# cvg/diffmvs

Measured on AMD Instinct MI355X. Metric: depth-maps/sec (640x512, 5 src views), higher is better.
Workload: dtype f32

## Files before the change

diffmvs_amd/_lib.py:

```python
from __future__ import annotations

import ctypes as C
import os

PKG = os.path.dirname(os.path.abspath(__file__))
HIP_LIB_PATH = os.environ.get("DMVS_LIB") or os.path.join(PKG, "libdmvs_hip.so")

ACT_NONE, ACT_RELU, ACT_SIGMOID, ACT_TANH, ACT_SILU = range(5)
IN_PLAIN, IN_UPSAMPLE2, IN_UNSHUFFLE2, IN_ZEROINSERT2 = range(4)
LAYOUT_NCHW, LAYOUT_NHWC, LAYOUT_NHWC_BF16, LAYOUT_NHWC_F16 = 0, 1, 2, 3
DTYPE_F32, DTYPE_BF16, DTYPE_F16, DTYPE_F32_PLAIN = 0, 1, 2, 3
ARITH_F32, ARITH_BF16, ARITH_SPLIT = 0, 1, 2
EW_DEPTH_TO_DISP, EW_DISP_TO_DEPTH = 0, 1

_P = C.c_void_p
_I = C.c_int32
_F = C.c_float


class Conv2dDesc(C.Structure):
    _fields_ = [
        ("in0", _P), ("in1", _P), ("mul0", _P), ("weight", _P), ("scale", _P), ("shift", _P),
        ("residual", _P), ("gru_z", _P), ("gru_h", _P), ("out", _P), ("gn_stats", _P), ("out_mul", _P),
        ("B", _I), ("c0", _I), ("c1", _I), ("Hin", _I), ("Win", _I), ("Hout", _I), ("Wout", _I),
        ("cout", _I), ("cout_pad", _I), ("kh", _I), ("kw", _I), ("stride", _I), ("pad_h", _I), ("pad_w", _I),
        ("in_mode", _I), ("act", _I), ("res_mode", _I), ("res_after_act", _I),
        ("out_layout", _I), ("out_cstride", _I), ("out_coffset", _I), ("gn_groups", _I), ("post_scale", _F),
        ("gate_cstride", _I), ("arith", _I), ("tune", _I), ("out_mul_c0", _I), ("in0_cstride", _I), ("weight_split", _P),
    ]


class Conv3dDesc(C.Structure):
    _fields_ = [
        ("in_", _P), ("weight", _P), ("scale", _P), ("shift", _P), ("residual", _P), ("out", _P),
        ("B", _I), ("cin", _I), ("cout", _I), ("cout_pad", _I),
        ("Din", _I), ("Hin", _I), ("Win", _I), ("Dout", _I), ("Hout", _I), ("Wout", _I),
        ("stride", _I), ("transposed", _I), ("act", _I), ("tune", _I),
    ]


class GetCostDesc(C.Structure):
    _fields_ = [
        ("ref", _P), ("src", _P), ("rt", _P), ("inv_depth", _P), ("confidence", _P), ("view_w", _P),
        ("disp_min", _P), ("disp_max", _P), ("out_cost", _P), ("out_samples", _P), ("worklist", _P),
        ("B", _I), ("S", _I), ("C", _I), ("G", _I), ("n", _I), ("H", _I), ("W", _I), ("vw_shift", _I),
        ("cost_cstride", _I), ("cost_coffset", _I), ("samp_cstride", _I), ("samp_coffset", _I),
        ("interval", _F), ("min_radius", _F), ("max_radius", _F), ("feat_dtype", _I), ("tune", _I),
    ]


SIGNATURES = {
    "dmvs_abi_version": [],
    "dmvs_conv2d_f32": [C.POINTER(Conv2dDesc), _P],
    "dmvs_featurenet_stem_f32": [_P, _P, _P, _P, _P, _P, _P, _P, _I, _I, _I, _I, _P],
    "dmvs_featurenet_stem3_f32": [_P, _P, _P, _P, _P, _P, _P, _P, _P, _P, _P, _I, _I, _I, _I, _P],
    "dmvs_featurenet_conv1_pair_f32": [_P, _P, _P, _P, _P, _P, _P, _P, _I, _I, _I, _I, _P],
    "dmvs_featurenet_fpn_tail_f32": [_P, _P, _P, _P, _P, _P, _I, _I, _I, _I, _P],
    "dmvs_conv2d_wgrad_workspace_f32": [C.POINTER(Conv2dDesc), C.POINTER(C.c_int64)],
    "dmvs_conv2d_wgrad_f32": [C.POINTER(Conv2dDesc), _P, _P, _P, _P, C.c_int64, _P],
    "dmvs_conv3d_f32": [C.POINTER(Conv3dDesc), _P],
    "dmvs_conv3d_wgrad_workspace_f32": [C.POINTER(Conv3dDesc), C.POINTER(C.c_int64)],
    "dmvs_conv3d_wgrad_f32": [C.POINTER(Conv3dDesc), _P, _P, _P, _P, C.c_int64, _P],
    "dmvs_compose_proj_f32": [_P, _P, _I, _I, _P],
    "dmvs_warp_volume_f32": [_P, _P, _P, _P, _I, _I, _I, _I, _I, _I, _I, _P],
    "dmvs_getcost_quad_f32": [C.POINTER(GetCostDesc), _P],
    "dmvs_warp_corr_init_quad_f32": [_P, _P, _P, _P, _P, _P, _I, _I, _I, _I, _I, _I, _I, _I, _I, _I, _I, _P],
    "dmvs_warp_corr_init_bwd_f32": [_P, _P, _P, _P, _P, _P, _P, _P, _I, _I, _I, _I, _I, _I, _I, _I, _I, _I, _P],
    "dmvs_getcost_bwd_f32": [C.POINTER(GetCostDesc), _P, _P, _P, _P],
    "dmvs_view_aggregate_bwd_f32": [_P, _P, _P, _P, _P, _P, _I, _I, _I, _I, _P],
    "dmvs_view_aggregate_f32": [_P, _P, _P, _I, _I, _I, _I, _P],
    "dmvs_sigmoid_max_d_f32": [_P, _P, _I, _I, _I, _P],
    "dmvs_depth_regress_f32": [_P, _P, _P, _P, _P, _P, _I, _I, _I, _P],
    "dmvs_convex_upsample_f32": [_P, _P, _P, _P, _P, _P, _I, _I, _I, _I, _P],
    "dmvs_mask_upsample4_f32": [_P, _P, _P, _F, _P, _P, _P, _P, _P, _I, _I, _I, _I, _I, _P],
    "dmvs_groupnorm_silu_f32": [_P, _P, _P, _P, _P, _P, _P, _I, _I, _I, _I, _F, _P],
    "dmvs_groupnorm_apply_f32": [_P, _P, _P, _P, _P, _P, _P, _I, _I, _I, _I, _F, _P],
# ... 96 lines not shown
```

diffmvs_amd/csrc/conv2d.hip:

```cpp
#include "conv2d_tiled.h"

namespace {

constexpr int kC11MaxCin = 64;

template <int NT, int OT, bool ACTX = false>
__global__ void __launch_bounds__(DMVS_BLOCK) conv1x1_px4_kernel(const dmvs_conv2d_desc d, int tiles_per_item) {
    constexpr int NW = NT * 16, WS = (NW % 32 == 0) ? NW + 16 : NW;
    __shared__ float s_w[kC11MaxCin * WS];
    DMVS_LDS_POISON(s_w);
    const int tid = threadIdx.x, lane = tid & 63, wave = tid >> 6;
    const int n = lane & 15, kq = lane >> 4;
    const int cin = d.c0 + d.c1, cin4 = (cin + 3) >> 2;
    const int HW = d.Hout * d.Wout;
    const int nbase = blockIdx.y * NW;
    for (int e = tid; e < cin4 * 4 * NW; e += DMVS_BLOCK) {
        const int k = e / NW, co = e - k * NW;
        s_w[k * WS + co] = (k < cin && nbase + co < d.cout_pad) ? d.weight[k * d.cout_pad + nbase + co] : 0.0f;
    }
    const int b = blockIdx.x / tiles_per_item, t = blockIdx.x - b * tiles_per_item;
    const int p = (t * 4 + wave) * 64 + 4 * n;
    const bool pok = p < HW;
    const int pcl = pok ? p : HW - 4;
    const float* in0b = d.in0 + (size_t)b * d.c0 * HW;
    const float* in1b = d.in1 ? d.in1 + (size_t)b * d.c1 * HW : d.in0;
    __syncthreads();

    f32x4 acc[4][NT];
#pragma unroll
    for (int r = 0; r < 4; ++r)
#pragma unroll
        for (int j = 0; j < NT; ++j) acc[r][j] = f32x4{0.0f, 0.0f, 0.0f, 0.0f};
    auto load = [&](int c) -> f32x4 {
        int ci = 4 * c + kq;
        ci = ci < cin ? ci : cin - 1;
        const float* src = ci < d.c0 ? in0b + (size_t)ci * HW : in1b + (size_t)(ci - d.c0) * HW;
        return *reinterpret_cast<const f32x4*>(src + pcl);
    };
    auto mma = [&](int c, const f32x4& x) {
        const bool ok = pok && 4 * c + kq < cin;
        const float* wp = s_w + (4 * c + kq) * WS + n;
        float xv[4];
#pragma unroll
        for (int r = 0; r < 4; ++r) xv[r] = ok ? x[r] : 0.0f;
#pragma unroll
        for (int nt = 0; nt < NT; ++nt) {
            const float aw = wp[nt * 16];
#pragma unroll
// ... 26 lines not shown
    for (int nt = 0; nt < NT; ++nt) {
        f32x4 y[4], res[4];
#pragma unroll
        for (int j = 0; j < 4; ++j) {
            const int cg = nbase + nt * 16 + 4 * kq + j;
            res[j] = f32x4{0.0f, 0.0f, 0.0f, 0.0f};
            if (resb && cg < d.cout) {
                if (rup) {
                    typedef float f32x2 __attribute__((ext_vector_type(2)));
                    const f32x2 rv = *reinterpret_cast<const f32x2*>(resb + (size_t)cg * rplane + rpix);
                    res[j] = f32x4{rv[0], rv[0], rv[1], rv[1]};
                } else {
                    res[j] = *reinterpret_cast<const f32x4*>(resb + (size_t)cg * HW + p);
                }
            }
        }
#pragma unroll
        for (int j = 0; j < 4; ++j) {
            const int cg = nbase + nt * 16 + 4 * kq + j;
            const bool okc = cg < d.cout;
            const float sc = d.scale ? d.scale[okc ? cg : 0] : 1.0f, sh = d.shift ? d.shift[okc ? cg : 0] : 0.0f;
#pragma unroll
            for (int r = 0; r < 4; ++r) y[j][r] = acc[r][nt][j] * sc + sh;
            if (!d.res_after_act) y[j] += res[j];
            if constexpr (ACTX) {
#pragma unroll
                for (int r = 0; r < 4; ++r) y[j][r] = dmvs_act(y[j][r], d.act);
            } else if (d.act == DMVS_ACT_RELU) {
#pragma unroll
                for (int r = 0; r < 4; ++r) y[j][r] = fmaxf(y[j][r], 0.0f);
            }
            y[j] *= d.post_scale;
            if (d.res_after_act) y[j] += res[j];
        }
        if constexpr (OT != DMVS_DTYPE_F32) {
            const int c0o = nbase + nt * 16 + 4 * kq;
            uint16_t* const ob = reinterpret_cast<uint16_t*>(d.out) + ((size_t)b * HW + p) * d.out_cstride + d.out_coffset + c0o;
#pragma unroll
            for (int r = 0; r < 4; ++r)
#pragma unroll
                for (int j = 0; j < 4; ++j)
                    if (c0o + j < d.cout) ob[(size_t)r * d.out_cstride + j] = dmvs_to_x16<OT>(y[j][r]);
        } else if (d.out_layout == DMVS_LAYOUT_NCHW) {
            float* const outb = d.out + ((size_t)b * d.out_cstride + d.out_coffset) * HW + p;
#pragma unroll
            for (int j = 0; j < 4; ++j) {
// ... 14 lines not shown
                        if (c0o + j < d.cout) ob[(size_t)r * d.out_cstride + j] = y[j][r];
                }
            }
        }
    }
}

static bool conv1x1_px4_ok(const dmvs_conv2d_desc& d) {
    if (d.kh != 1 || d.kw != 1 || d.stride != 1 || d.pad_h || d.pad_w || d.in_mode != DMVS_IN_PLAIN) return false;
    if (d.mul0 || d.gru_z || d.gn_stats || d.out_mul || d.in0_cstride || (d.tune & DMVS_TUNE_1X1_TILED)) return false;
    if (d.act > DMVS_ACT_RELU && (d.cout_pad > 16 || d.out_layout != DMVS_LAYOUT_NCHW)) return false;
    if (d.c0 + d.c1 > kC11MaxCin || d.cout_pad > 144 || (d.Wout & 3)) return false;
    if (d.res_mode == DMVS_IN_UPSAMPLE2 && ((d.Hout | d.Wout) & 1)) return false;
    if ((((uintptr_t)d.in0 | (uintptr_t)d.in1 | (uintptr_t)d.residual) & 15) != 0) return false;
    if (d.out_layout == DMVS_LAYOUT_NCHW && ((uintptr_t)d.out & 15)) return false;
    return true;
}

template <int NT>
static int launch_conv1x1_px4(const dmvs_conv2d_desc& d, hipStream_t st, int ngroups) {
    const int HW = d.Hout * d.Wout;
    const int tiles = (HW + 255) / 256;
    dim3 grid((unsigned)(tiles * d.B), (unsigned)ngroups), block(DMVS_BLOCK);
    if (d.out_layout == DMVS_LAYOUT_NHWC_BF16) hipLaunchKernelGGL((conv1x1_px4_kernel<NT, DMVS_DTYPE_BF16>), grid, block, 0, st, d, tiles);
    else if (d.out_layout == DMVS_LAYOUT_NHWC_F16) hipLaunchKernelGGL((conv1x1_px4_kernel<NT, DMVS_DTYPE_F16>), grid, block, 0, st, d, tiles);
    else hipLaunchKernelGGL((conv1x1_px4_kernel<NT, DMVS_DTYPE_F32>), grid, block, 0, st, d, tiles);
    return dmvs_launch_status();
}

static int conv1x1_px4(const dmvs_conv2d_desc& d, hipStream_t st) {
    if (d.act > DMVS_ACT_RELU) {
        const int HW = d.Hout * d.Wout, tiles = (HW + 255) / 256;
        hipLaunchKernelGGL((conv1x1_px4_kernel<1, DMVS_DTYPE_F32, true>), dim3((unsigned)(tiles * d.B)), dim3(DMVS_BLOCK), 0, st, d, tiles);
        return dmvs_launch_status();
    }
    const int ntiles = (d.cout_pad + 15) / 16;
    const int maxnt = d.residual ? 2 : 4;
    const int ngroups = (ntiles + maxnt - 1) / maxnt;
    const int nt = (ntiles + ngroups - 1) / ngroups;
    switch (nt) {
        case 1: return launch_conv1x1_px4<1>(d, st, ngroups);
        case 2: return launch_conv1x1_px4<2>(d, st, ngroups);
        case 3: return launch_conv1x1_px4<3>(d, st, ngroups);
        default: return launch_conv1x1_px4<4>(d, st, ngroups);
    }
}

template <int KH, int KW, int S, bool V16>
__global__ void __launch_bounds__(DMVS_BLOCK) conv2d_wgrad_kernel(const dmvs_conv2d_desc d, const float* __restrict__ gout,
                                                                  float* __restrict__ ws, int want_bias, int tiles_x, int tiles_y) {
    constexpr int T = KH * KW, CK = 8;
    constexpr int TW = 15 * S + KW, TH = 15 * S + KH;
    constexpr int SLACK = V16 ? (4 - ((KW - 1) / 2) % 4) % 4 : 0;
    constexpr int TWL = V16 ? (SLACK + TW + 3) / 4 * 4 : TW;
    constexpr int PLANE = pad16mod32(TH * TWL);
    constexpr int GROW = V16 ? 260 : 257;
    constexpr int NTN = (CK * T + 1 + 15) / 16;
    constexpr int IN_IT = ((V16 ? CK * PLANE / 4 : CK * PLANE) + DMVS_BLOCK - 1) / DMVS_BLOCK;
    constexpr int G_IT = ((V16 ? 16 * GROW / 4 : 16 * GROW) + DMVS_BLOCK - 1) / DMVS_BLOCK;
    __shared__ __attribute__((aligned(16))) float lds[CK * PLANE + 16 * GROW];
    DMVS_LDS_POISON(lds);
    float* s_in = lds;
    float* s_g = lds + CK * PLANE;

    const int tid = threadIdx.x, lane = tid & 63, wave = tid >> 6;
    const int m = lane & 15, kq = lane >> 4;
    const int c0 = blockIdx.y * CK, cobase = blockIdx.z * 16;
    const int cin = d.c0 + d.c1;
// ... 190 lines not shown
    g.floats = (long)g.gx * g.gy * g.gz * g.ntn * 256;
    return g;
}

template <int KH, int KW, int S>
int launch_wgrad(const dmvs_conv2d_desc& d, const float* gout, float* gw, float* gb, float* ws, hipStream_t st) {
    const int tiles_x = (d.Wout + 15) / 16, tiles_y = (d.Hout + 15) / 16;
    const WgradGrid g = wgrad_grid(d);
    const bool v16 = !(d.tune & DMVS_TUNE_PIECES4) && d.in_mode == DMVS_IN_PLAIN && !d.mul0 && (d.Win & 3) == 0 && (d.Wout & 3) == 0 &&
                     d.pad_w == (KW - 1) / 2 && (((uintptr_t)d.in0 | (uintptr_t)d.in1 | (uintptr_t)gout) & 15) == 0;
    if (v16)
        hipLaunchKernelGGL((conv2d_wgrad_kernel<KH, KW, S, true>), dim3(g.gx, g.gy, g.gz), dim3(DMVS_BLOCK), 0, st, d, gout, ws,
                           gb ? 1 : 0, tiles_x, tiles_y);
    else
    hipLaunchKernelGGL((conv2d_wgrad_kernel<KH, KW, S, false>), dim3(g.gx, g.gy, g.gz), dim3(DMVS_BLOCK), 0, st, d, gout, ws,
                       gb ? 1 : 0, tiles_x, tiles_y);
    hipLaunchKernelGGL((conv2d_wgrad_reduce_kernel<KH * KW>), dim3(g.ntn * 16, g.gy, g.gz), dim3(DMVS_BLOCK), 0, st, ws, gw, gb,
                       g.gx, g.gy, d.c0 + d.c1, d.cout, (d.tune & DMVS_TUNE_WGRAD_ACCUMULATE) ? 1 : 0);
    return dmvs_launch_status();
}

}

extern "C" int dmvs_conv2d_f32(const dmvs_conv2d_desc* dp, void* stream) {
    if (!dp) return DMVS_EINVAL;
    const dmvs_conv2d_desc& d = *dp;
    hipStream_t st = (hipStream_t)stream;
    if (d.cout_pad % 8 || d.cout > d.cout_pad || d.B <= 0 || !d.in0 || !d.weight || !d.out) return DMVS_EINVAL;
    if ((uintptr_t)d.weight & 15) return DMVS_EINVAL;
    if (d.c1 > 0 && (!d.in1 || d.in_mode != DMVS_IN_PLAIN)) return DMVS_EINVAL;
    if (d.mul0 && d.in_mode != DMVS_IN_PLAIN) return DMVS_EINVAL;
    if (d.in_mode == DMVS_IN_UNSHUFFLE2 && (d.c0 % 4)) return DMVS_EINVAL;
    if ((d.in_mode == DMVS_IN_UPSAMPLE2 || d.in_mode == DMVS_IN_ZEROINSERT2) && ((d.Hin | d.Win) & 1)) return DMVS_EINVAL;
    if (d.gru_z && (!d.gru_h || d.act != DMVS_ACT_TANH)) return DMVS_EINVAL;
    if (d.gate_cstride < 0 || (d.gate_cstride && d.in_mode != DMVS_IN_PLAIN)) return DMVS_EINVAL;
    if (d.in0_cstride < 0 || (d.in0_cstride && (d.in_mode != DMVS_IN_PLAIN || d.in0_cstride < d.c0))) return DMVS_EINVAL;
    if (d.out_mul && (d.out_mul_c0 < 0 || d.out_mul_c0 >= d.cout || d.gn_stats)) return DMVS_EINVAL;
    if (d.gn_stats && (d.gn_groups != 4 || d.cout % 4)) return DMVS_EINVAL;
    if (d.arith != DMVS_ARITH_F32 && d.arith != DMVS_ARITH_BF16 && d.arith != DMVS_ARITH_SPLIT) return DMVS_EINVAL;
    const int eh = (d.Hin + 2 * d.pad_h - d.kh) / d.stride + 1, ew = (d.Win + 2 * d.pad_w - d.kw) / d.stride + 1;
    if (eh != d.Hout || ew != d.Wout) return DMVS_EINVAL;
    if ((long)(d.c0 + d.c1) * d.Hin * d.Win * (d.in_mode == DMVS_IN_UNSHUFFLE2 ? 4 : 1) >= (1L << 31)) return DMVS_EINVAL;
    if (d.out_layout < DMVS_LAYOUT_NCHW || d.out_layout > DMVS_LAYOUT_NHWC_F16) return DMVS_EINVAL;
    if (d.out_layout >= DMVS_LAYOUT_NHWC_BF16 && (d.gru_z || d.gn_stats)) return DMVS_EINVAL;
    const int ocs = d.out_cstride > d.cout ? d.out_cstride : d.cout;
    if ((long)d.Hout * d.Wout >= (1L << 24) || ocs >= (1 << 24) || (long)ocs * d.Hout * d.Wout >= (1L << 31)) return DMVS_EINVAL;
    const int key = d.kh * 100 + d.kw * 10 + d.stride;
    switch (key) {
        case 111:
            return conv1x1_px4_ok(d) ? conv1x1_px4(d, st) : dmvs_detail::launch_conv2d_111(d, st);
        case 331: return dmvs_detail::launch_conv2d_331(d, st);
        case 332: return dmvs_detail::launch_conv2d_332(d, st);
        case 552: return dmvs_detail::launch_conv2d_552(d, st);
        case 551: return dmvs_detail::launch_conv2d_551(d, st);
        case 771: return dmvs_detail::launch_conv2d_771(d, st);
        case 151: return dmvs_detail::launch_conv2d_151(d, st);
        case 511: return dmvs_detail::launch_conv2d_511(d, st);
        default: return DMVS_EINVAL;
    }
}

static int wgrad_check(const dmvs_conv2d_desc& d) {
    if (d.cout_pad % 8 || d.cout > d.cout_pad || d.B <= 0 || !d.in0) return DMVS_EINVAL;
    if (d.c1 > 0 && (!d.in1 || d.in_mode != DMVS_IN_PLAIN)) return DMVS_EINVAL;
    if (d.mul0 && d.in_mode != DMVS_IN_PLAIN) return DMVS_EINVAL;
    if (d.in0_cstride || d.gate_cstride || d.out_mul) return DMVS_EINVAL;
    const int eh = (d.Hin + 2 * d.pad_h - d.kh) / d.stride + 1, ew = (d.Win + 2 * d.pad_w - d.kw) / d.stride + 1;
    if (eh != d.Hout || ew != d.Wout) return DMVS_EINVAL;
    return 0;
}

extern "C" int dmvs_conv2d_wgrad_workspace_f32(const dmvs_conv2d_desc* dp, int64_t* bytes) {
    if (!dp || !bytes) return DMVS_EINVAL;
    if (int rc = wgrad_check(*dp)) return rc;
    *bytes = (int64_t)wgrad_grid(*dp).floats * 4;
    return 0;
}

extern "C" int dmvs_conv2d_wgrad_f32(const dmvs_conv2d_desc* dp, const float* grad_out, float* gw, float* gb, float* workspace,
                                     int64_t workspace_bytes, void* stream) {
    if (!dp || !grad_out || !gw || !workspace) return DMVS_EINVAL;
    const dmvs_conv2d_desc& d = *dp;
// ... 16 lines not shown
```

diffmvs_amd/csrc/misc.hip:

```cpp
#include "dmvs_common.h"

extern "C" int dmvs_abi_version(void) { return DMVS_ABI_VERSION; }

__device__ static void build_cam(const float* pm, double (&P)[4][4]) {
    const float* E = pm;
    const float* K = pm + 16;
    for (int i = 0; i < 4; ++i)
        for (int j = 0; j < 4; ++j) P[i][j] = (double)E[i * 4 + j];
    for (int i = 0; i < 3; ++i)
        for (int j = 0; j < 4; ++j) {
            double a = 0.0;
            for (int k = 0; k < 3; ++k) a += (double)K[i * 4 + k] * (double)E[k * 4 + j];
            P[i][j] = a;
        }
}

__global__ void compose_proj_kernel(const float* __restrict__ proj, float* __restrict__ out, int B, int V) {
    const int S = V - 1;
    const int idx = blockIdx.x * blockDim.x + threadIdx.x;
    if (idx >= B * S) return;
    const int b = idx / S, s = idx % S;
    double R[4][4], A[4][8];
    build_cam(proj + ((size_t)b * V) * 32, R);
    for (int i = 0; i < 4; ++i)
// ... 217 lines not shown
    }
    __syncthreads();
    if (threadIdx.x == 0) {
        double a = 0.0, c = 0.0;
        for (int w = 0; w < DMVS_BLOCK / 64; ++w) {
            a += red[0][w];
            c += red[1][w];
        }
        dmvs_gn_accumulate(&stats[2 * bg], 0, a);
        dmvs_gn_accumulate(&stats[2 * bg], 1, c);
    }
}

constexpr int kGnPerLane = 16;

template <bool VEC>
__global__ void __launch_bounds__(DMVS_BLOCK)
gn_apply_kernel(const float* __restrict__ x, const float* __restrict__ gamma, const float* __restrict__ beta,
                const float* __restrict__ scale_shift, const float* __restrict__ residual, float* __restrict__ y,
                const double* __restrict__ stats, int C, int HW, int groups, float eps) {
    __shared__ float s_ab[2];
    const int bc = blockIdx.y;
    if (threadIdx.x == 0) {
        const int b = bc / C, c = bc % C;
        const int cg = C / groups;
        const int g = c / cg;
        const double n = (double)cg * HW;
        double s1, s2;
        dmvs_gn_read_pair(&stats[2 * (b * groups + g)], s1, s2);
        const double mean = s1 / n;
        double var = s2 / n - mean * mean;
        var = var < 0.0 ? 0.0 : var;
        const float rstd = (float)(1.0 / sqrt(var + (double)eps));
        float A = rstd * gamma[c];
        float Bc = beta[c] - (float)mean * A;
        if (scale_shift) {
            const float sc = scale_shift[(long)b * 2 * C + c] + 1.0f, sh = scale_shift[(long)b * 2 * C + C + c];
            A *= sc;
            Bc = Bc * sc + sh;
        }
        s_ab[0] = A;
        s_ab[1] = Bc;
    }
    __syncthreads();
    const float A = s_ab[0], Bc = s_ab[1];
    const long base = (long)bc * HW;
    const int i0 = blockIdx.x * (DMVS_BLOCK * kGnPerLane);
    if constexpr (VEC) {
        typedef float f32x4 __attribute__((ext_vector_type(4)));
#pragma unroll
        for (int k = 0; k < kGnPerLane / 4; ++k) {
            const int i = i0 + (k * DMVS_BLOCK + threadIdx.x) * 4;
            if (i < HW) {
                f32x4 v = *reinterpret_cast<const f32x4*>(x + base + i);
#pragma unroll
                for (int j = 0; j < 4; ++j) {
                    const float t = fmaf(v[j], A, Bc);
                    v[j] = t * dmvs_sigmoid(t);
                }
                if (residual) v += *reinterpret_cast<const f32x4*>(residual + base + i);
                *reinterpret_cast<f32x4*>(y + base + i) = v;
            }
        }
    } else {
#pragma unroll 4
        for (int k = 0; k < kGnPerLane; ++k) {
            const int i = i0 + k * DMVS_BLOCK + threadIdx.x;
            if (i < HW) {
                float v = fmaf(x[base + i], A, Bc);
                v = v * dmvs_sigmoid(v);
                if (residual) v += residual[base + i];
                y[base + i] = v;
            }
        }
    }
}

static void launch_gn_apply(const float* x, const float* gamma, const float* beta, const float* scale_shift, const float* residual,
                            float* y, const double* stats, int B, int C, int HW, int groups, float eps, hipStream_t st) {
    const dim3 grid(dmvs_ceil_div(HW, DMVS_BLOCK * kGnPerLane), (unsigned)(B * C));
    const bool vec = HW % 4 == 0 && (((uintptr_t)x | (uintptr_t)y | (uintptr_t)residual) & 15) == 0;
    if (vec) hipLaunchKernelGGL((gn_apply_kernel<true>), grid, dim3(DMVS_BLOCK), 0, st, x, gamma, beta, scale_shift, residual, y, stats, C, HW, groups, eps);
    else hipLaunchKernelGGL((gn_apply_kernel<false>), grid, dim3(DMVS_BLOCK), 0, st, x, gamma, beta, scale_shift, residual, y, stats, C, HW, groups, eps);
}

extern "C" int dmvs_groupnorm_silu_f32(const float* x, const float* gamma, const float* beta, const float* scale_shift,
                                       const float* residual, float* y, double* stats, int32_t B, int32_t C, int32_t HW,
                                       int32_t groups, float eps, void* stream) {
    if (!x || !y || !stats || groups <= 0 || C % groups) return DMVS_EINVAL;
    hipStream_t st = (hipStream_t)stream;
    hipError_t e = hipMemsetAsync(stats, 0, sizeof(double) * 2 * B * groups, st);
    if (e != hipSuccess) return (int)e;
    const long per_group = (long)(C / groups) * HW;
// ... 173 lines not shown
```

diffmvs_amd/engine.py:

```python
from __future__ import annotations

import math
import os
from typing import Callable, Dict, List, Optional

import torch
import torch.nn.functional as F

from . import ops as K
from .ops import Ops, PackedConv, pack_conv2d, pack_conv3d

_RATIOS = [4, 2, 1]
_MULTS = [(1,), (1, 2), (1, 2, 4)]


def _bn(sd, p):
    return {k: sd[f"{p}.{k}"] for k in ("weight", "bias", "running_mean", "running_var")}


def _cw(sd, p, **kw):
    return pack_conv2d(sd[p + ".conv.weight"], sd.get(p + ".conv.bias"),
                       bn=_bn(sd, p + ".bn") if (p + ".bn.weight") in sd else None, **kw)


# ... 174 lines not shown

    def reset(self, B):
        self.buf = self.bufs.get(B)
        if self.buf is None:
            self.buf = self.bufs[B] = torch.zeros(self.SLOTS, B * 8, dtype=torch.float64, device=self.ops.device)
        else:
            self.buf.zero_()
        self.next = 0

    def slot(self):
        if self.next >= self.SLOTS:
            raise RuntimeError("GroupNorm statistics arena exhausted")
        s = self.buf[self.next]
        self.next += 1
        return s


def run_resblock(o: Ops, arena: GnArena, rb, x0, x1=None, scale_shift=None):
    st1, st2 = arena.slot(), arena.slot()
    h = o.conv2d(rb["c1"], x0, x1, gn_stats=st1)
    h = o.groupnorm_apply(h, rb["g1"][0], rb["g1"][1], 4, st1, scale_shift=scale_shift, out=h)
    h2 = o.conv2d(rb["c2"], h, gn_stats=st2)
    if rb["res"] is not None:
        res = o.conv2d(rb["res"], x0, x1)
    else:
        assert x1 is None
        res = x0
    return o.groupnorm_apply(h2, rb["g2"][0], rb["g2"][1], 4, st2, residual=res, out=h2)


def run_unet(o: Ops, arena: GnArena, ub, E, ctx_part, hidden, ss_of):
    x = o.conv2d(ub.init_enc, E, residual=ctx_part)
    r = x
    skips = []
    L = len(ub.mults)
    for i, (blk, ds) in enumerate(ub.downs):
        x = run_resblock(o, arena, blk, x, None, ss_of(blk))
        skips.append(x)
        x = o.conv2d(ds, x, in_mode=(K.IN_UNSHUFFLE2 if i < L - 1 else K.IN_PLAIN))
    hidden = run_gru(o, ub.gru, hidden, x)
    x = run_resblock(o, arena, ub.mid, hidden, None, None)
    for i, (blk, us) in enumerate(ub.ups):
        x = run_resblock(o, arena, blk, x, skips.pop(), ss_of(blk))
        x = o.conv2d(us, x, in_mode=(K.IN_UPSAMPLE2 if i < L - 1 else K.IN_PLAIN))
    x = run_resblock(o, arena, ub.final, x, r, ss_of(ub.final))
    delta = o.conv2d(ub.final_conv, x)
# ... 355 lines not shown
```

diffmvs_amd/ops.py:

```python
from __future__ import annotations

import ctypes as C
import os
from dataclasses import dataclass
from typing import Optional

import torch

from . import _lib
from ._lib import (ACT_NONE, ACT_RELU, ACT_SIGMOID, ACT_SILU, ACT_TANH, ARITH_BF16, ARITH_F32, ARITH_SPLIT, DTYPE_BF16, DTYPE_F16, DTYPE_F32, IN_PLAIN,
                   IN_UNSHUFFLE2, IN_UPSAMPLE2, IN_ZEROINSERT2, LAYOUT_NCHW, LAYOUT_NHWC, LAYOUT_NHWC_BF16, LAYOUT_NHWC_F16)

CONV_ARITH = {"fp32": ARITH_F32, "bf16": ARITH_BF16, "split": ARITH_SPLIT}
FEATURE_DTYPES = {"fp32": torch.float32, "bf16": torch.bfloat16, "fp16": torch.float16}
_DTYPE_CODE = {torch.float32: DTYPE_F32, torch.bfloat16: DTYPE_BF16, torch.float16: DTYPE_F16}
_NHWC_LAYOUT = {torch.float32: LAYOUT_NHWC, torch.bfloat16: LAYOUT_NHWC_BF16, torch.float16: LAYOUT_NHWC_F16}


def _round_up(x: int, m: int) -> int:
    return (x + m - 1) // m * m


@dataclass
class PackedConv:
# ... 109 lines not shown
def bump_weights_generation() -> None:
    _weights_generation[0] += 1


BWD_INTERLEAVED_DEFAULT = 1


def _env_tune():
    e = os.environ.get
    t2 = _lib.tune_tile_wx(int(e("DMVS_CONV_WX", "0"))) | _lib.tune_tile_mt(int(e("DMVS_CONV_MT", "0")))
    t2 |= _lib.TUNE_NO_WALK if e("DMVS_CONV_WALK") == "0" else 0
    t2 |= _lib.TUNE_PIECES4 if e("DMVS_CONV_V16") == "0" else 0
    t2 |= _lib.TUNE_NO_LEAN if e("DMVS_CONV_LEAN") == "0" else 0
    t2 |= _lib.TUNE_1X1_TILED if e("DMVS_CONV1X1_PX4") == "0" else 0
    t2 |= {"0": _lib.TUNE_NO_TALL, "1": _lib.TUNE_TALL}.get(e("DMVS_CONV_TALL"), 0)
    t2 |= _lib.TUNE_SPLIT_ALL if e("DMVS_CONV_SPLIT_ALL") == "1" else 0
    t2 |= _lib.tune_xcd_group(int(e("DMVS_CONV_XCD", "0")))
    t3 = (_lib.TUNE3D_PIECES4 if e("DMVS_CONV3D_V16") == "0" else 0) | (_lib.TUNE3D_S2_DIRECT if e("DMVS_CONV3D_S2") == "direct" else 0)
    t3 |= _lib.TUNE3D_NO_PAIR if e("DMVS_CONV3D_PAIR") == "0" else 0
    t3 |= _lib.tune3d_xcd_group(int(e("DMVS_CONV3D_XCD", "0")))
    return {"conv2d": t2, "conv3d": t3, "stem": (_lib.TUNE_PIECES4 if e("DMVS_STEM_V16") == "0" else 0) | _lib.tune_xcd_group(int(e("DMVS_STEM_XCD", "0"))) | (_lib.TUNE_STEM_EXACT if e("DMVS_STEM_EXACT") == "1" else 0),
            "sweep": _lib.TUNE_SWEEP_GLOBAL if e("DMVS_PLANE_SWEEP") == "quad" else 0,
            "bwd_gather": e("DMVS_GETCOST_BWD") == "gather",
            "bwd_il": e("DMVS_BWD_INTERLEAVED", "%d" % BWD_INTERLEAVED_DEFAULT) == "1"}


class Ops:
    _bindings = {}

    def __init__(self, lib: _lib.Lib, device):
        self.lib = lib
        self.device = torch.device(device)
        self.tune = _env_tune()
        self.timers = None
        self.conv_arith = ARITH_F32
        self.debug_fill = None
        self.getcost_hook = None

    def with_conv_arith(self, arith: int) -> "Ops":
        import copy
        o = copy.copy(self)
        o.conv_arith = arith
        return o

    def _call(self, name, *args):
        if self.timers is not None and name in self.timers:
            st, en = torch.cuda.Event(enable_timing=True), torch.cuda.Event(enable_timing=True)
            st.record()
            self.lib.call(name, *args)
            en.record()
            self.timers[name].append((st, en))
        else:
            self.lib.call(name, *args)

    @classmethod
    def for_device(cls, device) -> "Ops":
        device = torch.device(device)
        if device.type != "cuda":
            raise _lib.DmvsError(
                f"diffmvs_amd runs on MI355X only (got device '{device}'); there is no CPU path. "
                "Move the model and inputs to a HIP device.")
        if device.index is None:
            device = torch.device("cuda", torch.cuda.current_device())
        lib = _lib.hip_lib()
        key = (lib.path, device.index)
        o = cls._bindings.get(key)
        if o is None:
            o = cls._bindings[key] = cls(lib, device)
        return o

    def stream(self):
        if self.device.type == "cuda":
            return C.c_void_p(torch.cuda.current_stream(self.device).cuda_stream)
        return None
# ... 14 lines not shown
        dt = ts[0].dtype
        for t in ts:
            if t.dtype not in _DTYPE_CODE or t.dtype != dt or not t.is_contiguous() or t.device != self.device:
                raise _lib.DmvsError(f"expected contiguous fp32 / bf16 / fp16 feature tensors of one dtype on {self.device}, got "
                                     f"{t.dtype} contiguous={t.is_contiguous()} on {t.device}")
        return _DTYPE_CODE[dt]

    def _chk(self, *ts):
        for t in ts:
            if t is None:
                continue
            if t.dtype != torch.float32 or not t.is_contiguous() or t.device != self.device:
                raise _lib.DmvsError(f"expected contiguous fp32 tensor on {self.device}, got {t.dtype} "
                                     f"contiguous={t.is_contiguous()} on {t.device}")

    def _chk_typed(self, what, *pairs):
        for t, dt in pairs:
            if t is not None and (t.dtype != dt or not t.is_contiguous() or t.device != self.device):
                raise _lib.DmvsError(f"{what}: expected a contiguous {dt} tensor on {self.device}, got {t.dtype} on {t.device}")

    def conv2d(self, pc: PackedConv, x0, x1=None, *, mul0=None, in_mode=IN_PLAIN, act=ACT_NONE, residual=None,
               res_mode=IN_PLAIN, res_after_act=False, post_scale=1.0, gru_z=None, gru_h=None, out=None,
               out_layout=LAYOUT_NCHW, out_cstride=None, out_coffset=0, gn_stats=None, gn_groups=4, out_dtype=torch.float32,
               gate_cstride=0, arith=None, tune=None, out_mul=None, out_mul_c0=0, in0_cstride=0):
        if in0_cstride:
            if (x0.dtype != torch.float32 or x0.device != self.device or x0.stride(1) != x0.shape[2] * x0.shape[3] or
                    x0.stride(0) != in0_cstride * x0.shape[2] * x0.shape[3] or x0.stride(3) != 1 or in_mode != IN_PLAIN):
                raise _lib.DmvsError("in0_cstride: x0 must be a channel slice of a contiguous [B,in0_cstride,H,W] tensor, plain input mode")
        self._chk(out_mul)
        if gate_cstride:
            self._chk(*(() if in0_cstride else (x0,)), x1, residual, gru_h)
            for t in (mul0, gru_z):
                if t is not None and (t.dtype != torch.float32 or t.device != self.device or t.stride(1) != t.shape[2] * t.shape[3] or
                                      t.stride(0) != gate_cstride * t.shape[2] * t.shape[3] or t.stride(3) != 1):
                    raise _lib.DmvsError("gate_cstride: mul0 / gru_z must be channel slices of a contiguous [B,gate_cstride,H,W] tensor")
        else:
            self._chk(*(() if in0_cstride else (x0,)), x1, mul0, residual, gru_z, gru_h)
        if out_dtype != torch.float32:
            if out_layout != LAYOUT_NHWC or out is not None:
                raise _lib.DmvsError("16-bit outputs are channel-last feature tensors allocated by conv2d")
            out_layout = _NHWC_LAYOUT[out_dtype]
        else:
            self._chk(out)
        if gn_stats is not None and (gn_stats.dtype != torch.float64 or gn_stats.numel() < x0.shape[0] * gn_groups * 2):
            raise _lib.DmvsError("gn_stats must be float64 with B*groups*2 elements")
        B = x0.shape[0]
        if in_mode == IN_PLAIN:
# ... 4 lines not shown
            c0, Hin, Win = x0.shape[1] * 4, x0.shape[2] // 2, x0.shape[3] // 2
        c1 = 0 if x1 is None else x1.shape[1]
        assert c0 + c1 == pc.cin, (c0, c1, pc.cin)
        kh, kw = pc.k
        Hout = (Hin + 2 * pc.pad[0] - kh) // pc.stride + 1
        Wout = (Win + 2 * pc.pad[1] - kw) // pc.stride + 1
        if out_cstride is None:
            out_cstride = pc.cout
        if out is None:
            shape = (B, out_cstride, Hout, Wout) if out_layout == LAYOUT_NCHW else (B, Hout, Wout, out_cstride)
            out = self.empty(*shape, dtype=out_dtype)
        arith = self.conv_arith if arith is None else arith
        wsplit = split_weights(pc) if (arith == ARITH_SPLIT and kh * kw > 1 and out_layout in (LAYOUT_NCHW, LAYOUT_NHWC)) else None
        d = _lib.Conv2dDesc(
            weight_split=_ptr(wsplit),
            in0=_ptr(x0), in1=_ptr(x1), mul0=_ptr(mul0), weight=_ptr(pc.weight), scale=_ptr(pc.scale),
            shift=_ptr(pc.shift), residual=_ptr(residual), gru_z=_ptr(gru_z), gru_h=_ptr(gru_h), out=_ptr(out),
            gn_stats=_ptr(gn_stats), gn_groups=(gn_groups if gn_stats is not None else 0), B=B, c0=c0, c1=c1, Hin=Hin, Win=Win, Hout=Hout, Wout=Wout, cout=pc.cout, cout_pad=pc.cout_pad,
            kh=kh, kw=kw, stride=pc.stride, pad_h=pc.pad[0], pad_w=pc.pad[1], in_mode=in_mode, act=act,
            res_mode=res_mode, res_after_act=int(res_after_act), out_layout=out_layout, out_cstride=out_cstride,
            out_coffset=out_coffset, post_scale=post_scale, gate_cstride=gate_cstride,
            arith=arith, tune=(self.tune["conv2d"] if tune is None else tune),
            out_mul=_ptr(out_mul), out_mul_c0=out_mul_c0, in0_cstride=in0_cstride)
        self._call("dmvs_conv2d_f32", C.byref(d), self.stream())
        if self.timers is not None and "dmvs_conv2d_f32" in self.timers:
            self.timers.setdefault("_conv2d_flops", []).append(2.0 * B * Hout * Wout * pc.cout * pc.cin * kh * kw)
            self.timers.setdefault("_conv2d_shape", []).append((B, pc.cin, pc.cout, kh, kw, pc.stride, Hout, Wout, in_mode, int(mul0 is not None)))
            nb = sum(t.numel() * t.element_size() for t in (x0, x1, mul0, residual, gru_z, gru_h, out_mul) if t is not None)
            self.timers.setdefault("_conv2d_bytes", []).append(nb + B * Hout * Wout * pc.cout * out.element_size())
        return out

    def featurenet_stem(self, pc0: PackedConv, pc1: PackedConv, x, tune=None):
        if isinstance(x, (list, tuple)):
            self._chk(*x)
            Bv, cin, H, W = x[0].shape
            y = self.empty(len(x) * Bv, 8, H, W)
            for v, xv in enumerate(x):
                self._stem_launch(pc0, pc1, xv, y[v * Bv:(v + 1) * Bv], tune)
            return y
        self._chk(x)
        N, cin, H, W = x.shape
        y = self.empty(N, 8, H, W)
        self._stem_launch(pc0, pc1, x, y, tune)
        return y

    def _stem_launch(self, pc0: PackedConv, pc1: PackedConv, x, y, tune=None):
        N, cin, H, W = x.shape
# ... 683 lines not shown
```

include/dmvs.h:

```cpp
#ifndef DMVS_H
#define DMVS_H

#include <stdint.h>

#ifdef __cplusplus
extern "C" {
#endif

#define DMVS_ABI_VERSION 4
#define DMVS_EINVAL (-22)

enum { DMVS_ACT_NONE = 0, DMVS_ACT_RELU = 1, DMVS_ACT_SIGMOID = 2, DMVS_ACT_TANH = 3, DMVS_ACT_SILU = 4 };
enum { DMVS_IN_PLAIN = 0, DMVS_IN_UPSAMPLE2 = 1 , DMVS_IN_UNSHUFFLE2 = 2 ,
       DMVS_IN_ZEROINSERT2 = 3  };
enum { DMVS_LAYOUT_NCHW = 0, DMVS_LAYOUT_NHWC = 1,
       DMVS_LAYOUT_NHWC_BF16 = 2, DMVS_LAYOUT_NHWC_F16 = 3 };
enum { DMVS_DTYPE_F32 = 0 , DMVS_DTYPE_BF16 = 1, DMVS_DTYPE_F16 = 2 ,
       DMVS_DTYPE_F32_PLAIN = 3  };

int dmvs_abi_version(void);

#define DMVS_ARITH_F32 0
#define DMVS_ARITH_BF16 1
#define DMVS_ARITH_SPLIT 2
// ... 23 lines not shown
    double* gn_stats;
    const float* out_mul;
    int32_t B, c0, c1;
    int32_t Hin, Win;
    int32_t Hout, Wout;
    int32_t cout, cout_pad;
    int32_t kh, kw, stride, pad_h, pad_w;
    int32_t in_mode, act;
    int32_t res_mode;
    int32_t res_after_act;
    int32_t out_layout, out_cstride, out_coffset;
    int32_t gn_groups;
    float post_scale;
    int32_t gate_cstride;
    int32_t arith;
    int32_t tune;
    int32_t out_mul_c0;
    int32_t in0_cstride;
    const void* weight_split;
} dmvs_conv2d_desc;

int dmvs_conv2d_f32(const dmvs_conv2d_desc* d, void* stream);

int dmvs_featurenet_stem_f32(const float* x, const float* w0, const float* scale0, const float* shift0, const float* w1,
                             const float* scale1, const float* shift1, float* y, int32_t N, int32_t H, int32_t W, int32_t tune,
                             void* stream);

int dmvs_featurenet_stem3_f32(const float* x, const float* w0, const float* scale0, const float* shift0, const float* w1,
                              const float* scale1, const float* shift1, const float* w2, const float* scale2, const float* shift2,
                              float* y, int32_t N, int32_t H, int32_t W, int32_t tune, void* stream);

int dmvs_featurenet_conv1_pair_f32(const float* x, const void* wsplit1, const float* scale1, const float* shift1, const void* wsplit2,
                                   const float* scale2, const float* shift2, float* y, int32_t N, int32_t H, int32_t W, int32_t tune,
                                   void* stream);

int dmvs_featurenet_fpn_tail_f32(const float* c2, const float* c3, const float* w_inner, const float* b_inner, const void* wsplit_out,
                                 float* y, int32_t N, int32_t H, int32_t W, int32_t tune, void* stream);

#define DMVS_TUNE_WGRAD_ACCUMULATE 0x1000
int dmvs_conv2d_wgrad_workspace_f32(const dmvs_conv2d_desc* d, int64_t* bytes);
int dmvs_conv2d_wgrad_f32(const dmvs_conv2d_desc* d, const float* grad_out, float* gw, float* gb, float* workspace,
                          int64_t workspace_bytes, void* stream);

typedef struct dmvs_conv3d_desc {
    const float* in;
    const float* weight;
// ... 211 lines not shown
```

Measured before the change: 1547.

## Fuse GroupNorm+SiLU of residual branch into the 1x1 shortcut conv epilogue

Adds a GN-aware variant of the 1x1 conv kernel that builds per-channel GroupNorm affine coefficients in shared memory and applies GN+SiLU to the residual operand in the epilogue, writing in place over h2. In the residual block this replaces a separate shortcut conv, a groupnorm_apply pass and a residual-add read/write with a single kernel, saving one full feature-map round trip through memory. The fused path is enabled by default through a tune flag and only taken when alignment and shape checks pass. In exchange the epilogue recomputes GN coefficients per workgroup and each element pays a sigmoid.

Result: no change. 1553, median of 4 (+0.4%).

```diff
diff --git a/diffmvs_amd/_lib.py b/diffmvs_amd/_lib.py
--- a/diffmvs_amd/_lib.py
+++ b/diffmvs_amd/_lib.py
@@ -30,6 +30,10 @@
     ]
 
 
+class GnOperand(C.Structure):
+    _fields_ = [("stats", _P), ("gamma", _P), ("beta", _P), ("scale_shift", _P), ("groups", _I), ("eps", _F)]
+
+
 class Conv3dDesc(C.Structure):
     _fields_ = [
         ("in_", _P), ("weight", _P), ("scale", _P), ("shift", _P), ("residual", _P), ("out", _P),
@@ -52,6 +56,7 @@
 SIGNATURES = {
     "dmvs_abi_version": [],
     "dmvs_conv2d_f32": [C.POINTER(Conv2dDesc), _P],
+    "dmvs_conv2d_gn_f32": [C.POINTER(Conv2dDesc), C.POINTER(GnOperand), _P],
     "dmvs_featurenet_stem_f32": [_P, _P, _P, _P, _P, _P, _P, _P, _I, _I, _I, _I, _P],
     "dmvs_featurenet_stem3_f32": [_P, _P, _P, _P, _P, _P, _P, _P, _P, _P, _P, _I, _I, _I, _I, _P],
     "dmvs_featurenet_conv1_pair_f32": [_P, _P, _P, _P, _P, _P, _P, _P, _I, _I, _I, _I, _P],
diff --git a/diffmvs_amd/csrc/conv2d.hip b/diffmvs_amd/csrc/conv2d.hip
--- a/diffmvs_amd/csrc/conv2d.hip
+++ b/diffmvs_amd/csrc/conv2d.hip
@@ -1,11 +1,14 @@
 #include "conv2d_tiled.h"
+#include "dmvs_gn.h"
 
 namespace {
 
 constexpr int kC11MaxCin = 64;
 
-template <int NT, int OT, bool ACTX = false>
-__global__ void __launch_bounds__(DMVS_BLOCK) conv1x1_px4_kernel(const dmvs_conv2d_desc d, int tiles_per_item) {
+struct conv_no_gn {};
+template <int NT, int OT, bool ACTX = false, bool GNR = false>
+__global__ void __launch_bounds__(DMVS_BLOCK) conv1x1_px4_kernel(const dmvs_conv2d_desc d, int tiles_per_item,
+                                                                 const std::conditional_t<GNR, dmvs_gn_operand, conv_no_gn> gn) {
     constexpr int NW = NT * 16, WS = (NW % 32 == 0) ? NW + 16 : NW;
     __shared__ float s_w[kC11MaxCin * WS];
     DMVS_LDS_POISON(s_w);
@@ -24,6 +27,14 @@
     const int pcl = pok ? p : HW - 4;
     const float* in0b = d.in0 + (size_t)b * d.c0 * HW;
     const float* in1b = d.in1 ? d.in1 + (size_t)b * d.c1 * HW : d.in0;
+    [[maybe_unused]] const float* s_gn = nullptr;
+    if constexpr (GNR) {
+        __shared__ float s_gn_tab[2 * DMVS_GN_TABLE];
+        static_assert(NW <= DMVS_GN_TABLE, "one table slot per output channel of the workgroup");
+        DMVS_LDS_POISON(s_gn_tab);
+        dmvs_gn_fill_table(s_gn_tab, gn, b, nbase, NW, d.cout, HW, tid);
+        s_gn = s_gn_tab;
+    }
     __syncthreads();
 
     f32x4 acc[4][NT];
@@ -96,6 +107,11 @@
             const float sc = d.scale ? d.scale[okc ? cg : 0] : 1.0f, sh = d.shift ? d.shift[okc ? cg : 0] : 0.0f;
 #pragma unroll
             for (int r = 0; r < 4; ++r) y[j][r] = acc[r][nt][j] * sc + sh;
+            if constexpr (GNR) {
+                const float ga = s_gn[nt * 16 + 4 * kq + j], gb = s_gn[DMVS_GN_TABLE + nt * 16 + 4 * kq + j];
+#pragma unroll
+                for (int r = 0; r < 4; ++r) res[j][r] = okc ? dmvs_gn_silu(res[j][r], ga, gb) : 0.0f;
+            }
             if (!d.res_after_act) y[j] += res[j];
             if constexpr (ACTX) {
 #pragma unroll
@@ -156,16 +172,16 @@
     const int HW = d.Hout * d.Wout;
     const int tiles = (HW + 255) / 256;
     dim3 grid((unsigned)(tiles * d.B), (unsigned)ngroups), block(DMVS_BLOCK);
-    if (d.out_layout == DMVS_LAYOUT_NHWC_BF16) hipLaunchKernelGGL((conv1x1_px4_kernel<NT, DMVS_DTYPE_BF16>), grid, block, 0, st, d, tiles);
-    else if (d.out_layout == DMVS_LAYOUT_NHWC_F16) hipLaunchKernelGGL((conv1x1_px4_kernel<NT, DMVS_DTYPE_F16>), grid, block, 0, st, d, tiles);
-    else hipLaunchKernelGGL((conv1x1_px4_kernel<NT, DMVS_DTYPE_F32>), grid, block, 0, st, d, tiles);
+    if (d.out_layout == DMVS_LAYOUT_NHWC_BF16) hipLaunchKernelGGL((conv1x1_px4_kernel<NT, DMVS_DTYPE_BF16>), grid, block, 0, st, d, tiles, conv_no_gn{});
+    else if (d.out_layout == DMVS_LAYOUT_NHWC_F16) hipLaunchKernelGGL((conv1x1_px4_kernel<NT, DMVS_DTYPE_F16>), grid, block, 0, st, d, tiles, conv_no_gn{});
+    else hipLaunchKernelGGL((conv1x1_px4_kernel<NT, DMVS_DTYPE_F32>), grid, block, 0, st, d, tiles, conv_no_gn{});
     return dmvs_launch_status();
 }
 
 static int conv1x1_px4(const dmvs_conv2d_desc& d, hipStream_t st) {
     if (d.act > DMVS_ACT_RELU) {
         const int HW = d.Hout * d.Wout, tiles = (HW + 255) / 256;
-        hipLaunchKernelGGL((conv1x1_px4_kernel<1, DMVS_DTYPE_F32, true>), dim3((unsigned)(tiles * d.B)), dim3(DMVS_BLOCK), 0, st, d, tiles);
+        hipLaunchKernelGGL((conv1x1_px4_kernel<1, DMVS_DTYPE_F32, true>), dim3((unsigned)(tiles * d.B)), dim3(DMVS_BLOCK), 0, st, d, tiles, conv_no_gn{});
         return dmvs_launch_status();
     }
     const int ntiles = (d.cout_pad + 15) / 16;
@@ -178,6 +194,15 @@
         case 3: return launch_conv1x1_px4<3>(d, st, ngroups);
         default: return launch_conv1x1_px4<4>(d, st, ngroups);
     }
+}
+
+static int conv1x1_px4_gn_res(const dmvs_conv2d_desc& d, const dmvs_gn_operand& gn, hipStream_t st) {
+    const int ntiles = (d.cout_pad + 15) / 16, ngroups = (ntiles + 1) / 2, nt = (ntiles + ngroups - 1) / ngroups;
+    const int HW = d.Hout * d.Wout, tiles = (HW + 255) / 256;
+    const dim3 grid((unsigned)(tiles * d.B), (unsigned)ngroups), block(DMVS_BLOCK);
+    if (nt == 1) hipLaunchKernelGGL((conv1x1_px4_kernel<1, DMVS_DTYPE_F32, false, true>), grid, block, 0, st, d, tiles, gn);
+    else hipLaunchKernelGGL((conv1x1_px4_kernel<2, DMVS_DTYPE_F32, false, true>), grid, block, 0, st, d, tiles, gn);
+    return dmvs_launch_status();
 }
 
 template <int KH, int KW, int S, bool V16>
@@ -414,10 +439,7 @@
 
 }
 
-extern "C" int dmvs_conv2d_f32(const dmvs_conv2d_desc* dp, void* stream) {
-    if (!dp) return DMVS_EINVAL;
-    const dmvs_conv2d_desc& d = *dp;
-    hipStream_t st = (hipStream_t)stream;
+static int conv2d_check(const dmvs_conv2d_desc& d) {
     if (d.cout_pad % 8 || d.cout > d.cout_pad || d.B <= 0 || !d.in0 || !d.weight || !d.out) return DMVS_EINVAL;
     if ((uintptr_t)d.weight & 15) return DMVS_EINVAL;
     if (d.c1 > 0 && (!d.in1 || d.in_mode != DMVS_IN_PLAIN)) return DMVS_EINVAL;
@@ -437,6 +459,14 @@
     if (d.out_layout >= DMVS_LAYOUT_NHWC_BF16 && (d.gru_z || d.gn_stats)) return DMVS_EINVAL;
     const int ocs = d.out_cstride > d.cout ? d.out_cstride : d.cout;
     if ((long)d.Hout * d.Wout >= (1L << 24) || ocs >= (1 << 24) || (long)ocs * d.Hout * d.Wout >= (1L << 31)) return DMVS_EINVAL;
+    return 0;
+}
+
+extern "C" int dmvs_conv2d_f32(const dmvs_conv2d_desc* dp, void* stream) {
+    if (!dp) return DMVS_EINVAL;
+    const dmvs_conv2d_desc& d = *dp;
+    hipStream_t st = (hipStream_t)stream;
+    if (const int e = conv2d_check(d)) return e;
     const int key = d.kh * 100 + d.kw * 10 + d.stride;
     switch (key) {
         case 111:
@@ -450,6 +480,20 @@
         case 511: return dmvs_detail::launch_conv2d_511(d, st);
         default: return DMVS_EINVAL;
     }
+}
+
+static bool gn_operand_ok(const dmvs_gn_operand& g, int C) {
+    return g.stats && g.gamma && g.beta && g.groups > 0 && C % g.groups == 0 && !((uintptr_t)g.stats & 7);
+}
+
+extern "C" int dmvs_conv2d_gn_f32(const dmvs_conv2d_desc* dp, const dmvs_gn_operand* gn_res, void* stream) {
+    if (!gn_res) return dmvs_conv2d_f32(dp, stream);
+    if (!dp) return DMVS_EINVAL;
+    const dmvs_conv2d_desc& d = *dp;
+    if (const int e = conv2d_check(d)) return e;
+    if (d.out_layout != DMVS_LAYOUT_NCHW || d.act > DMVS_ACT_RELU || !d.residual || d.res_mode != DMVS_IN_PLAIN) return DMVS_EINVAL;
+    if (!gn_operand_ok(*gn_res, d.cout) || !conv1x1_px4_ok(d)) return DMVS_EINVAL;
+    return conv1x1_px4_gn_res(d, *gn_res, (hipStream_t)stream);
 }
 
 static int wgrad_check(const dmvs_conv2d_desc& d) {
diff --git a/diffmvs_amd/csrc/dmvs_gn.h b/diffmvs_amd/csrc/dmvs_gn.h
--- /dev/null
+++ b/diffmvs_amd/csrc/dmvs_gn.h
@@ -0,0 +1,41 @@
+#pragma once
+#include "dmvs_common.h"
+
+__device__ __forceinline__ void dmvs_gn_coeffs(const double* __restrict__ stats, const float* __restrict__ gamma, const float* __restrict__ beta,
+                                               const float* __restrict__ scale_shift, int b, int c, int C, int HW, int groups, float eps,
+                                               float& A_out, float& Bc_out) {
+    const int cg = C / groups;
+    const int g = c / cg;
+    const double n = (double)cg * HW;
+    double s1, s2;
+    dmvs_gn_read_pair(&stats[2 * (b * groups + g)], s1, s2);
+    const double mean = s1 / n;
+    double var = s2 / n - mean * mean;
+    var = var < 0.0 ? 0.0 : var;
+    const float rstd = (float)(1.0 / sqrt(var + (double)eps));
+    float A = rstd * gamma[c];
+    float Bc = beta[c] - (float)mean * A;
+    if (scale_shift) {
+        const float sc = scale_shift[(long)b * 2 * C + c] + 1.0f, sh = scale_shift[(long)b * 2 * C + C + c];
+        A *= sc;
+        Bc = Bc * sc + sh;
+    }
+    A_out = A;
+    Bc_out = Bc;
+}
+
+__device__ __forceinline__ float dmvs_gn_silu(float x, float A, float Bc) {
+#pragma clang fp contract(off)
+    const float t = fmaf(x, A, Bc);
+    return t * dmvs_sigmoid(t);
+}
+
+#define DMVS_GN_TABLE 64
+__device__ __forceinline__ void dmvs_gn_fill_table(float* tab, const dmvs_gn_operand& g, int b, int c_first, int nch, int C, int HW, int tid) {
+    if (tid < nch && c_first + tid < C) {
+        float A, Bc;
+        dmvs_gn_coeffs(g.stats, g.gamma, g.beta, g.scale_shift, b, c_first + tid, C, HW, g.groups, g.eps, A, Bc);
+        tab[tid] = A;
+        tab[DMVS_GN_TABLE + tid] = Bc;
+    }
+}
diff --git a/diffmvs_amd/csrc/misc.hip b/diffmvs_amd/csrc/misc.hip
--- a/diffmvs_amd/csrc/misc.hip
+++ b/diffmvs_amd/csrc/misc.hip
@@ -1,4 +1,5 @@
 #include "dmvs_common.h"
+#include "dmvs_gn.h"
 
 extern "C" int dmvs_abi_version(void) { return DMVS_ABI_VERSION; }
 
@@ -263,23 +264,8 @@
     __shared__ float s_ab[2];
     const int bc = blockIdx.y;
     if (threadIdx.x == 0) {
-        const int b = bc / C, c = bc % C;
-        const int cg = C / groups;
-        const int g = c / cg;
-        const double n = (double)cg * HW;
-        double s1, s2;
-        dmvs_gn_read_pair(&stats[2 * (b * groups + g)], s1, s2);
-        const double mean = s1 / n;
-        double var = s2 / n - mean * mean;
-        var = var < 0.0 ? 0.0 : var;
-        const float rstd = (float)(1.0 / sqrt(var + (double)eps));
-        float A = rstd * gamma[c];
-        float Bc = beta[c] - (float)mean * A;
-        if (scale_shift) {
-            const float sc = scale_shift[(long)b * 2 * C + c] + 1.0f, sh = scale_shift[(long)b * 2 * C + C + c];
-            A *= sc;
-            Bc = Bc * sc + sh;
-        }
+        float A, Bc;
+        dmvs_gn_coeffs(stats, gamma, beta, scale_shift, bc / C, bc % C, C, HW, groups, eps, A, Bc);
         s_ab[0] = A;
         s_ab[1] = Bc;
     }
@@ -295,10 +281,7 @@
             if (i < HW) {
                 f32x4 v = *reinterpret_cast<const f32x4*>(x + base + i);
 #pragma unroll
-                for (int j = 0; j < 4; ++j) {
-                    const float t = fmaf(v[j], A, Bc);
-                    v[j] = t * dmvs_sigmoid(t);
-                }
+                for (int j = 0; j < 4; ++j) v[j] = dmvs_gn_silu(v[j], A, Bc);
                 if (residual) v += *reinterpret_cast<const f32x4*>(residual + base + i);
                 *reinterpret_cast<f32x4*>(y + base + i) = v;
             }
@@ -308,8 +291,7 @@
         for (int k = 0; k < kGnPerLane; ++k) {
             const int i = i0 + k * DMVS_BLOCK + threadIdx.x;
             if (i < HW) {
-                float v = fmaf(x[base + i], A, Bc);
-                v = v * dmvs_sigmoid(v);
+                float v = dmvs_gn_silu(x[base + i], A, Bc);
                 if (residual) v += residual[base + i];
                 y[base + i] = v;
             }
diff --git a/diffmvs_amd/engine.py b/diffmvs_amd/engine.py
--- a/diffmvs_amd/engine.py
+++ b/diffmvs_amd/engine.py
@@ -220,6 +220,8 @@
     h = o.groupnorm_apply(h, rb["g1"][0], rb["g1"][1], 4, st1, scale_shift=scale_shift, out=h)
     h2 = o.conv2d(rb["c2"], h, gn_stats=st2)
     if rb["res"] is not None:
+        if (o.tune.get("gn_fuse", 0) & 2) and K.conv_gn_res_eligible(rb["res"], x0, x1, residual=h2, tune=o.tune["conv2d"]):
+            return o.conv2d(rb["res"], x0, x1, residual=h2, gn_res=(st2, rb["g2"][0], rb["g2"][1], 4, None), out=h2)
         res = o.conv2d(rb["res"], x0, x1)
     else:
         assert x1 is None
diff --git a/diffmvs_amd/ops.py b/diffmvs_amd/ops.py
--- a/diffmvs_amd/ops.py
+++ b/diffmvs_amd/ops.py
@@ -155,7 +155,21 @@
     return {"conv2d": t2, "conv3d": t3, "stem": (_lib.TUNE_PIECES4 if e("DMVS_STEM_V16") == "0" else 0) | _lib.tune_xcd_group(int(e("DMVS_STEM_XCD", "0"))) | (_lib.TUNE_STEM_EXACT if e("DMVS_STEM_EXACT") == "1" else 0),
             "sweep": _lib.TUNE_SWEEP_GLOBAL if e("DMVS_PLANE_SWEEP") == "quad" else 0,
             "bwd_gather": e("DMVS_GETCOST_BWD") == "gather",
-            "bwd_il": e("DMVS_BWD_INTERLEAVED", "%d" % BWD_INTERLEAVED_DEFAULT) == "1"}
+            "bwd_il": e("DMVS_BWD_INTERLEAVED", "%d" % BWD_INTERLEAVED_DEFAULT) == "1",
+            "gn_fuse": int(e("DMVS_GN_FUSE", "%d" % GN_FUSE_DEFAULT))}
+
+
+def _aligned16(*ts):
+    return all(t is None or t.data_ptr() % 16 == 0 for t in ts)
+
+
+def conv_gn_res_eligible(pc: PackedConv, x0, x1=None, groups=4, act=ACT_NONE, residual=None, out=None, tune=0) -> bool:
+    return (tuple(pc.k) == (1, 1) and pc.stride == 1 and tuple(pc.pad) == (0, 0) and pc.cin <= 64 and pc.cout_pad <= 144 and pc.cout % groups == 0 and
+            x0.shape[3] % 4 == 0 and act in (ACT_NONE, ACT_RELU) and not (tune & _lib.TUNE_1X1_TILED) and residual is not None and
+            _aligned16(x0, x1, residual, out))
+
+
+GN_FUSE_DEFAULT = 2
 
 
 class Ops:
@@ -176,13 +190,14 @@
         o.conv_arith = arith
         return o
 
-    def _call(self, name, *args):
-        if self.timers is not None and name in self.timers:
+    def _call(self, name, *args, timer_key=None):
+        key = timer_key or name
+        if self.timers is not None and key in self.timers:
             st, en = torch.cuda.Event(enable_timing=True), torch.cuda.Event(enable_timing=True)
             st.record()
             self.lib.call(name, *args)
             en.record()
-            self.timers[name].append((st, en))
+            self.timers[key].append((st, en))
         else:
             self.lib.call(name, *args)
 
@@ -243,7 +258,7 @@
     def conv2d(self, pc: PackedConv, x0, x1=None, *, mul0=None, in_mode=IN_PLAIN, act=ACT_NONE, residual=None,
                res_mode=IN_PLAIN, res_after_act=False, post_scale=1.0, gru_z=None, gru_h=None, out=None,
                out_layout=LAYOUT_NCHW, out_cstride=None, out_coffset=0, gn_stats=None, gn_groups=4, out_dtype=torch.float32,
-               gate_cstride=0, arith=None, tune=None, out_mul=None, out_mul_c0=0, in0_cstride=0):
+               gate_cstride=0, arith=None, tune=None, out_mul=None, out_mul_c0=0, in0_cstride=0, gn_res=None, gn_eps=1e-5):
         if in0_cstride:
             if (x0.dtype != torch.float32 or x0.device != self.device or x0.stride(1) != x0.shape[2] * x0.shape[3] or
                     x0.stride(0) != in0_cstride * x0.shape[2] * x0.shape[3] or x0.stride(3) != 1 or in_mode != IN_PLAIN):
@@ -294,7 +309,14 @@
             out_coffset=out_coffset, post_scale=post_scale, gate_cstride=gate_cstride,
             arith=arith, tune=(self.tune["conv2d"] if tune is None else tune),
             out_mul=_ptr(out_mul), out_mul_c0=out_mul_c0, in0_cstride=in0_cstride)
-        self._call("dmvs_conv2d_f32", C.byref(d), self.stream())
+        if gn_res is None:
+            self._call("dmvs_conv2d_f32", C.byref(d), self.stream())
+        else:
+            stats, gamma, beta, groups, ss = gn_res
+            self._chk(gamma, beta, ss)
+            self._chk_typed("GroupNorm statistics", (stats, torch.float64))
+            g = _lib.GnOperand(stats=_ptr(stats), gamma=_ptr(gamma), beta=_ptr(beta), scale_shift=_ptr(ss), groups=groups, eps=gn_eps)
+            self._call("dmvs_conv2d_gn_f32", C.byref(d), C.byref(g), self.stream(), timer_key="dmvs_conv2d_f32")
         if self.timers is not None and "dmvs_conv2d_f32" in self.timers:
             self.timers.setdefault("_conv2d_flops", []).append(2.0 * B * Hout * Wout * pc.cout * pc.cin * kh * kw)
             self.timers.setdefault("_conv2d_shape", []).append((B, pc.cin, pc.cout, kh, kw, pc.stride, Hout, Wout, in_mode, int(mul0 is not None)))
diff --git a/include/dmvs.h b/include/dmvs.h
--- a/include/dmvs.h
+++ b/include/dmvs.h
@@ -69,6 +69,17 @@
 
 int dmvs_conv2d_f32(const dmvs_conv2d_desc* d, void* stream);
 
+typedef struct dmvs_gn_operand {
+    const double* stats;
+    const float* gamma;
+    const float* beta;
+    const float* scale_shift;
+    int32_t groups;
+    float eps;
+} dmvs_gn_operand;
+
+int dmvs_conv2d_gn_f32(const dmvs_conv2d_desc* d, const dmvs_gn_operand* gn_res, void* stream);
+
 int dmvs_featurenet_stem_f32(const float* x, const float* w0, const float* scale0, const float* shift0, const float* w1,
                              const float* scale1, const float* shift1, float* y, int32_t N, int32_t H, int32_t W, int32_t tune,
                              void* stream);
```
